# rapidsai/cugraph-gnn

Measured on AMD Instinct MI355X. Metric: sampled-edges/sec (sample+renumber+feature-gather+SAGEConv fwd), ogbn-products-like fan-out [25, 10], higher is better.
Workload: dtype int64 ids (int32 timed as a variant) + f32 features (SAGE lin_l/lin_r product: bf16x3-split MFMA, f32 accumulate); 1 GPU; ogbn-products-like RMAT: V=2449029, E=118462496 directed (CSR row_ptr i64 / col i64 replicated per GPU), feat fp32 [V,100], batch 1024/GPU, fan-out [25, 10], 2-layer SAGEConv(mean) 100-256-47 fwd, step = 8 call groups of 188 mini-batches; parallelism=dp1 (seeds sharded, no data-path collective)

## Files before the change

cugraph-gnn_amd/csrc/wg_append_unique.hip:

```cpp
#include <algorithm>
#include <type_traits>

#include "wg_common.hpp"

namespace wgamd {
namespace {

constexpr int kEmptyPos = 0x7fffffff;

template <typename KeyT>
struct key_traits;
template <>
struct key_traits<int32_t> {
  using cas_t                             = unsigned int;
  static constexpr wholememory_dtype_t dt = WHOLEMEMORY_DT_INT;
};
template <>
struct key_traits<int64_t> {
  using cas_t                             = unsigned long long;
  static constexpr wholememory_dtype_t dt = WHOLEMEMORY_DT_INT64;
};

__device__ __forceinline__ uint32_t hash_key(uint64_t k)
{
// ... 285 lines not shown
  table_clear_packed_kernel<<<(int)std::min<int64_t>(ceil_div(slots, 1024), 4096), 256, 0, stream>>>(table, slots, T, E);
  if (P > 0)
    table_insert_packed_kernel<TgtT, NbrT><<<ceil_div(P, 256), 256, 0, stream>>>(targets, T, neighbors, E, bv, table, slots, lay,
                                                                                 slot_of);
  if (E.host > 0) first_flag_packed_kernel<<<ceil_div(E.host, 256), 256, 0, stream>>>(table, slot_of, T, E, lay, rank);
  WG_HIP_CHECK(hipGetLastError());
  exclusive_scan_i32(rank, rank, E.host, scan_tmp, stream, E.dev);
}

#ifndef WG_LDS_SLOTS
#define WG_LDS_SLOTS 10000
#define WG_LDS_KEYS 3000
#define WG_LDS_THREADS 512
#define WG_LDS_UNROLL 7
#endif
constexpr int kLdsSlots      = WG_LDS_SLOTS;
constexpr int kLdsKeysTarget = WG_LDS_KEYS;
constexpr int kLdsProbeLimit = 256;
constexpr int kLdsThreads    = WG_LDS_THREADS;
constexpr int kLdsMaxRanges  = 2048;
constexpr int kLdsStack      = 40;
constexpr int kLdsChunks     = 16;
constexpr int kBucketThreads = 256;
constexpr int kBucketUnroll  = 4;
constexpr int kLdsUnroll     = WG_LDS_UNROLL;

__device__ __forceinline__ uint32_t hash_id32(uint32_t h)
{
  h ^= h >> 16;
  h *= 0x85ebca6bu;
  h ^= h >> 13;
  h *= 0xc2b2ae35u;
  return h ^ (h >> 16);
}
template <bool ID32>
__device__ __forceinline__ uint32_t hash_id(int64_t id)
{
  if constexpr (ID32) return hash_id32((uint32_t)id);
  else return hash_key((uint64_t)id);
}

struct batch_part {
  int t0, nT, e0, nE, P, R, rb, chunk;
  __device__ batch_part(const batch_view& bv, int b, int keys_target)
  {
    t0 = bv.target_seg[b];
// ... 5 lines not shown
    rb = (t0 + e0) / keys_target + 2 * b;
    chunk = (P + kLdsChunks - 1) / kLdsChunks;
  }
};

__device__ __forceinline__ bool batch_of_block(int G, int parts, int& b, int& part)
{
  const int x = blockIdx.x & 7, y = blockIdx.x >> 3;
  b    = (y / parts) * 8 + x;
  part = y % parts;
  return b < G;
}
inline int batch_grid(int G, int parts) { return 8 * ((G + 7) / 8) * parts; }

struct sort_scratch {
  int keys_target;
  int* seg_off;
  unsigned long long* words;
};

template <typename TgtT, typename NbrT>
__global__ void __launch_bounds__(kBucketThreads)
bucket_sort_kernel(const TgtT* __restrict__ targets, dev_count T_, const NbrT* __restrict__ neighbors, batch_view bv,
                   packed_layout lay, sort_scratch sc)
{
  constexpr bool ID32  = sizeof(NbrT) == 4;
  constexpr int kItems = kLdsMaxRanges / kBucketThreads;
  __shared__ int hist[kLdsMaxRanges];
  __shared__ int wave_tot[kBucketThreads / 64];
  int b, c;
  if (!batch_of_block(bv.G, kLdsChunks, b, c)) return;
  const batch_part bp(bv, b, sc.keys_target);
  if (bp.nE <= 0) return;
  const int T = T_.get(), tid = threadIdx.x;
  for (int r = tid; r < bp.R; r += kBucketThreads) hist[r] = 0;
  __syncthreads();
  const int begin = min(c * bp.chunk, bp.P), end = min(bp.P, begin + bp.chunk);
  const TgtT* tg = targets + bp.t0;
  const NbrT* nb = neighbors + bp.e0 - bp.nT;
  for (int i0 = begin + tid; i0 < end; i0 += kBucketThreads * kBucketUnroll) {
    int64_t id[kBucketUnroll];
#pragma unroll
    for (int k = 0; k < kBucketUnroll; k++) {
      const int i = min(i0 + k * kBucketThreads, end - 1);
      id[k]       = i < bp.nT ? (int64_t)tg[i] : (int64_t)nb[i];
    }
#pragma unroll
    for (int k = 0; k < kBucketUnroll; k++)
      if (i0 + k * kBucketThreads < end) atomicAdd(&hist[__umulhi(hash_id<ID32>(id[k]), (uint32_t)bp.R)], 1);
  }
  __syncthreads();
  {
// ... 31 lines not shown
  unsigned long long* out = sc.words + (bp.t0 + bp.e0) + begin;
  for (int i0 = begin + tid; i0 < end; i0 += kBucketThreads * kBucketUnroll) {
    int64_t id[kBucketUnroll];
#pragma unroll
    for (int k = 0; k < kBucketUnroll; k++) {
      const int i = min(i0 + k * kBucketThreads, end - 1);
      id[k]       = i < bp.nT ? (int64_t)tg[i] : (int64_t)nb[i];
    }
#pragma unroll
    for (int k = 0; k < kBucketUnroll; k++) {
      const int i = i0 + k * kBucketThreads;
      if (i < end) {
        const int dst = atomicAdd(&hist[__umulhi(hash_id<ID32>(id[k]), (uint32_t)bp.R)], 1);
        const int pos = i < bp.nT ? bp.t0 + i : T + bp.e0 + (i - bp.nT);
        out[dst]      = ((unsigned long long)id[k] << lay.pos_bits) | (unsigned long long)pos;
      }
    }
  }
}

template <bool ID32>
__global__ void __launch_bounds__(kLdsThreads)
renumber_lds_kernel(dev_count T_, dev_count E_, batch_view bv, packed_layout lay, int wg_per_batch, sort_scratch sc,
                    int* __restrict__ slot_of, int* __restrict__ tile_sums, int n_tile_sums)
{
  __shared__ unsigned long long tbl[kLdsSlots];
  __shared__ unsigned long long st_lo[kLdsStack], st_span[kLdsStack];
  __shared__ int st_n, overfull;
  __shared__ int seg_base[kLdsChunks], seg_pre[kLdsChunks + 1];
  const unsigned long long kEmpty = ~0ull;
  const int T = T_.get();
  const int tid = threadIdx.x;
  if (blockIdx.x == 0) {
    for (int i = tid; i < n_tile_sums; i += kLdsThreads) tile_sums[i] = 0;
  }
  int b, j;
  if (!batch_of_block(bv.G, wg_per_batch, b, j)) return;
  const batch_part bp(bv, b, sc.keys_target);
  if (bp.nE <= 0) return;
  const unsigned long long pos_mask = lay.pos_mask();
  const volatile int* overfull_now  = &overfull;
  static_assert(kLdsChunks == 16, "the segment search below is written for 16 segments");

  for (int r = j; r < bp.R; r += wg_per_batch) {
    __syncthreads();
    if (tid < kLdsChunks) {
      const int* row = sc.seg_off + (int64_t)(bp.rb + r) * kLdsChunks;
      const int lo = row[tid], n = row[kLdsChunks + tid] - lo;
      seg_base[tid] = bp.t0 + bp.e0 + tid * bp.chunk + lo;
      int inc = n;
#pragma unroll
      for (int d = 1; d < kLdsChunks; d <<= 1) {
        const int up = __shfl_up(inc, d, 64);
        if (tid >= d) inc += up;
      }
      seg_pre[tid + 1] = inc;
      if (tid == 0) {
        seg_pre[0] = 0;
        const unsigned long long lo_h = (((unsigned long long)r << 32) + bp.R - 1) / (unsigned)bp.R;
        st_lo[0]   = lo_h;
        st_span[0] = ((((unsigned long long)(r + 1) << 32) + bp.R - 1) / (unsigned)bp.R) - lo_h;
        st_n       = 1;
// ... 62 lines not shown
            memo[k] = (int)s;
          }
        }
      }
      __syncthreads();
      if (overfull) {
        if (tid == 0) {
          const unsigned long long half = span / 2;
          const int m = st_n;
          if (span < 2 || m + 2 > kLdsStack) __builtin_trap();
          st_lo[m]       = lo + half;
          st_span[m]     = span - half;
          st_lo[m + 1]   = lo;
          st_span[m + 1] = half;
          st_n           = m + 2;
        }
        __syncthreads();
        continue;
      }
      if (one_trip) {
#pragma unroll
        for (int k = 0; k < kLdsUnroll; k++) {
          const int p = (int)(w[k] & pos_mask);
          if (memo[k] >= 0 && p >= T) slot_of[p] = (int)(tbl[memo[k]] & pos_mask);
        }
        __syncthreads();
        continue;
      }
      for (int i0 = 0; i0 < n_pairs; i0 += kLdsThreads * kLdsUnroll) {
        if (!one_trip) {
#pragma unroll
          for (int k = 0; k < kLdsUnroll; k++) w[k] = pair_at(i0 + k * kLdsThreads + tid);
        }
#pragma unroll
        for (int k = 0; k < kLdsUnroll; k++) {
          const unsigned long long word = w[k];
          const unsigned long long id   = word >> lay.pos_bits;
          const int p                   = (int)(word & pos_mask);
          const uint32_t h              = hash_id<ID32>((int64_t)id);
          if (word != kEmpty && p >= T && (unsigned long long)h - lo < span) {
            uint32_t s = __umulhi(h * 0x9E3779B1u, (uint32_t)kLdsSlots);
            unsigned long long cur = tbl[s];
            while ((cur >> lay.pos_bits) != id) {
              s   = s + 1 == (uint32_t)kLdsSlots ? 0u : s + 1;
              cur = tbl[s];
            }
            slot_of[p] = (int)(cur & pos_mask);
          }
        }
      }
      __syncthreads();
    }
  }
}

struct rank_array {
  const int* rank;
  __device__ __forceinline__ int at(int q) const { return rank[q]; }
  __device__ __forceinline__ int total(int , int e_host) const { return rank[e_host]; }
};
struct rank_bits {
  const int* prefix;
  const unsigned long long* words;
  __device__ __forceinline__ int at(int q) const
  {
    const int w = q >> 6;
    return prefix[w] + __popcll(words[w] & ((1ull << (q & 63)) - 1ull));
  }
  __device__ __forceinline__ int total(int e_live, int ) const { return at(e_live); }
};
struct rank_bits_layout {
  int nw;
  int words_at;
  int live_at;
  __host__ __device__ explicit rank_bits_layout(int e_host)
// ... 105 lines not shown
    for (int k = 0; k < kEmitUnroll; k++) row[k] = first[k] < T ? first[k] + shift : tail_row + rank.at(first[k] - T);
#pragma unroll
    for (int k = 0; k < kEmitUnroll; k++) {
      const int i = i0 + k * 256;
      if (i >= end) break;
      const int e = e0 + i;
      if (first[k] == T + e) {
        const KeyT id      = (KeyT)neighbors[e];
        unique_out[row[k]] = id;
        if (bv.unique_batch) bv.unique_batch[row[k]] = b;
        if (bv.frontier_out) {
          const int r = row[k] - tail_row;
          static_cast<KeyT*>(bv.frontier_out)[r] = id;
          bv.frontier_batch_out[r]               = b;
        }
      }
      if (map_out) map_out[e] = row[k];
      if (bv.neighbor_local_out) bv.neighbor_local_out[e] = row[k] - (t0 + shift);
      if (bv.center_local_out) bv.center_local_out[e] = bv.edge_row[e] - s0 + local0;
    }
  }
}

inline int64_t lds_range_records(int64_t capacity_positions, int G) { return capacity_positions / kLdsKeysTarget + 3 * (int64_t)G + 2; }
inline int lds_keys_target()
{
  static const int v = [] {
    const char* e = getenv("WGAMD_RENUMBER_KEYS_TARGET");
    const long t  = e ? atol(e) : 0;
    return t > kLdsKeysTarget ? (int)std::min<long>(t, 1 << 30) : kLdsKeysTarget;
  }();
  return v;
}
inline bool lds_scratch_fits(int64_t capacity_positions, int G, int64_t slots)
{
  return 8 * capacity_positions + 256 <= 8 * slots && lds_range_records(capacity_positions, G) * kLdsChunks <= slots;
}

inline bool lds_path_taken(dev_count T, dev_count E, bool nbr64, const batch_view& bv, int64_t slots, packed_layout& lay)
{
  static const bool no_lds = getenv("WGAMD_RENUMBER_NO_LDS") != nullptr;
  const int64_t bound = bv.id_bound > 0 ? bv.id_bound : (nbr64 ? 0 : ((int64_t)1 << 31));
  const bool batched  = bv.target_batch != nullptr;
  return batched && !no_lds && bv.target_seg && bv.edge_offsets && bv.G > 1 && E.host >= 64 &&
         rank_bits_layout(E.host).ints() <= E.host + 1 &&
         packed_layout_for((int64_t)T.host + E.host, 1, bound, lay) && lds_scratch_fits((int64_t)T.host + E.host, bv.G, slots);
}

template <typename TgtT, typename NbrT>
void prepare_lds_t(const TgtT* targets, dev_count T, const NbrT* neighbors, dev_count E, batch_view bv, packed_layout lay,
                   void* keys, int* minpos, int* slot_of, int* rank, int* scan_tmp, hipStream_t stream)
{
  if (E.host > 0) {
    const int64_t cap = (int64_t)T.host + E.host;
    sort_scratch sc;
    sc.keys_target = lds_keys_target();
    sc.seg_off     = minpos;
    sc.words       = static_cast<unsigned long long*>(keys);
    bucket_sort_kernel<TgtT, NbrT><<<batch_grid(bv.G, kLdsChunks), kBucketThreads, 0, stream>>>(targets, T, neighbors, bv, lay, sc);
    const int64_t per_batch = (cap + bv.G - 1) / bv.G;
    const int wg_per_batch  = (int)std::max<int64_t>(1, std::min<int64_t>((per_batch + kLdsKeysTarget - 1) / kLdsKeysTarget, 32));
    const rank_bits_layout rl(E.host);
    const int n_tiles = (int)((rl.nw + kScanTile - 1) / kScanTile);
    renumber_lds_kernel<sizeof(NbrT) == 4><<<batch_grid(bv.G, wg_per_batch), kLdsThreads, 0, stream>>>(T, E, bv, lay, wg_per_batch, sc,
                                                                                                     slot_of, scan_tmp, n_tiles);
    const int bits_grid = (int)std::min<int64_t>(((int64_t)rl.nw + kBitsWordsPerBlock - 1) / kBitsWordsPerBlock, 256 * 8);
    first_bits_kernel<<<bits_grid, 256, 0, stream>>>(slot_of, T, E, rank, scan_tmp);
    WG_HIP_CHECK(hipGetLastError());
    exclusive_scan_i32_presummed(rank, rank, rl.nw, scan_tmp, stream, rank + rl.live_at);
  }
}

template <typename TgtT, typename NbrT, typename TableKeyT>
void prepare_t(const TgtT* targets, dev_count T, const NbrT* neighbors, dev_count E, batch_view bv, TableKeyT* keys,
               int* minpos, int64_t slots, int* slot_of, int* rank, int* scan_tmp, hipStream_t stream)
{
  const int P = T.host + E.host;
  table_clear_kernel<TableKeyT><<<(int)std::min<int64_t>(ceil_div(slots, 1024), 4096), 256, 0, stream>>>(keys, minpos, slots, T,
                                                                                                   E);
  if (P > 0)
    table_insert_kernel<TgtT, NbrT, TableKeyT><<<ceil_div(P, 256), 256, 0, stream>>>(targets, T, neighbors, E, bv, keys,
                                                                                    minpos, slots, slot_of);
  if (E.host > 0) first_flag_kernel<<<ceil_div(E.host, 256), 256, 0, stream>>>(minpos, slot_of, T, E, rank);
  WG_HIP_CHECK(hipGetLastError());
  exclusive_scan_i32(rank, rank, E.host, scan_tmp, stream, E.dev);
}

template <typename F>
// ... 38 lines not shown
    if constexpr (sizeof(TgtT) == 4) {
      if (!batched) {
        prepare_t<int32_t, int32_t, int32_t>(t, T, n, E, bv, static_cast<int32_t*>(keys), minpos, slots, slot_of, rank, scan_tmp, stream);
        return;
      }
    }
    prepare_t(t, T, n, E, bv, static_cast<int64_t*>(keys), minpos, slots, slot_of, rank, scan_tmp, stream);
  });
}

void append_unique_emit_enqueue(const void* targets, dev_count T, bool tgt64, const void* neighbors, dev_count E, bool nbr64,
                                batch_view bv, const int* minpos, const int* slot_of, const int* rank, int64_t slots,
                                void* unique_out, int* map_out, int* counts_out, hipStream_t stream)
{
  packed_layout lay_unused{};
  const bool bits = lds_path_taken(T, E, nbr64, bv, slots, lay_unused);
  const int P    = T.host + E.host;
  const int grid = ceil_div(P > bv.G + 1 ? P : bv.G + 1, 256);
  const bool per_batch = bv.target_batch != nullptr && bv.target_seg && bv.edge_offsets && bv.G > 1;
  const int bgrid = std::max(batch_grid(bv.G, kEmitChunks), ceil_div(bv.G + 1, 256));
  with_id_types(tgt64, nbr64, targets, neighbors, [&](auto* t, auto* n) {
    using TgtT = std::remove_cv_t<std::remove_pointer_t<decltype(t)>>;
    using NbrT = std::remove_cv_t<std::remove_pointer_t<decltype(n)>>;
    if (per_batch && bits) {
      const rank_bits_layout rl(E.host);
      const rank_bits rb{rank, reinterpret_cast<const unsigned long long*>(rank + rl.words_at)};
      renumber_emit_batched_kernel<TgtT, NbrT, rank_bits><<<bgrid, 256, 0, stream>>>(t, n, slot_of, rb, T, E, bv,
                                                                                    static_cast<TgtT*>(unique_out), map_out, counts_out);
    } else if (per_batch)
      renumber_emit_batched_kernel<TgtT, NbrT, rank_array><<<bgrid, 256, 0, stream>>>(t, n, slot_of, rank_array{rank}, T, E, bv,
                                                                                     static_cast<TgtT*>(unique_out), map_out, counts_out);
    else
      renumber_emit_kernel<TgtT, NbrT><<<grid, 256, 0, stream>>>(t, n, minpos, slot_of, rank, T, E, bv, static_cast<TgtT*>(unique_out),
                                                                map_out, counts_out);
  });
  WG_HIP_CHECK(hipGetLastError());
}

}

extern "C" {

wholememory_error_code_t graph_append_unique(wholememory_tensor_t target_nodes_tensor,
                                             wholememory_tensor_t neighbor_nodes_tensor,
                                             void* output_unique_node_memory_context,
                                             wholememory_tensor_t output_neighbor_raw_to_unique_mapping_tensor,
                                             wholememory_env_func_t* p_env_fns, void* stream)
// ... 61 lines not shown
```

cugraph-gnn_amd/csrc/wg_common.hpp:

```cpp
#pragma once
#include <hip/hip_runtime.h>

#include <cstdarg>
#include <cstdint>
#include <cstdio>
#include <stdexcept>
#include <vector>
#include <mutex>
#include <string>
#include <unordered_map>

#include "wgamd_ops.h"
#include "wgamd_tensor.h"
#include "wgamd_types.h"

struct wholememory_tensor_ {
  void* storage_ptr;
  wholememory_tensor_description_t desc;
  wholememory_tensor_* root;
  wholememory_handle_t handle;
  bool owns_handle = false;
  uint64_t handle_serial = 0;
};

// ... 255 lines not shown
                             const void* seeds, bool seeds64, dev_count n, int M, rng_plan random_seed, const int* offsets,
                             int* big_list, uint32_t* slab, int64_t slab_len, void* dst, int* src_lid,
                             int64_t* edge_gid, hipStream_t stream);
int64_t append_unique_slots(int64_t capacity);
struct batch_view {
  const int* target_batch;
  const int* target_seg;
  const int* edge_row;
  const int* edge_offsets;
  int G;
  int64_t id_bound;
  int* unique_batch;
  int* unique_seg;
  const int* sample_batch;
  const int* sample_seg;
  const int* sample_local0;
  void* frontier_out;
  int* frontier_batch_out;
  int* frontier_seg_out;
  int* frontier_local0_out;
  int* neighbor_local_out;
  int* center_local_out;
  int no_pad;
  __host__ __device__ const int* sbatch() const { return sample_batch ? sample_batch : target_batch; }
  __host__ __device__ const int* sseg() const { return sample_seg ? sample_seg : target_seg; }
};
void append_unique_prepare_enqueue(const void* targets, dev_count T, bool tgt64, const void* neighbors, dev_count E, bool nbr64,
                                   batch_view bv, void* keys, int* minpos, int64_t slots, int* slot_of, int* rank,
                                   int* scan_tmp, hipStream_t stream);
void append_unique_emit_enqueue(const void* targets, dev_count T, bool tgt64, const void* neighbors, dev_count E, bool nbr64,
                                batch_view bv, const int* minpos, const int* slot_of, const int* rank, int64_t slots,
                                void* unique_out, int* map_out, int* counts_out ,
                                hipStream_t stream);


void local_rows_gather(const char* table, wholememory_matrix_description_t tm, const void* idx,
                       wholememory_dtype_t idx_dtype, int64_t n, char* out, wholememory_matrix_description_t om,
                       hipStream_t stream);
void local_rows_scatter(const char* in, wholememory_matrix_description_t im, const void* idx,
                        wholememory_dtype_t idx_dtype, int64_t n, char* table, wholememory_matrix_description_t tm,
                        hipStream_t stream);
void local_rows_permute(const char* src, wholememory_matrix_description_t sm, const int64_t* src_idx, const int64_t* dst_idx,
                        int64_t n, char* dst, wholememory_matrix_description_t dm, hipStream_t stream);
struct id_exchange {
  wholememory_comm_t comm = nullptr;
  int W = 1, me = 0;
// ... 28 lines not shown
```

cugraph-gnn_amd/csrc/wg_fused.hip:

```cpp
#include <atomic>

#include "wg_common.hpp"
#include "wgamd_ext.h"

namespace wgamd {
namespace {

inline size_t align_up(size_t v) { return (v + 255) & ~(size_t)255; }

struct hop_workspace {
  size_t cnt, scan_tmp, nbr, keys, minpos, slot_of, rank, big_list, slab, row_start, row_deg, loc_hist, total;
  int64_t slots, slab_len;
};

hop_workspace plan(int64_t target_cap, int64_t edge_cap, size_t id_bytes, bool batched, int64_t max_row_len = 0)
{
  hop_workspace w{};
  size_t off = 0;
  auto take  = [&](size_t bytes) {
    size_t at = off;
    off += align_up(bytes);
    return at;
  };
  w.slots        = append_unique_slots(target_cap + edge_cap);
// ... 463 lines not shown

wholememory_error_code_t wgamd_sample_hop_batched_nosync(
  const int64_t* csr_row_ptr, const void* csr_col, wholememory_dtype_t id_dtype, const void* targets,
  const int* target_batch, const int* target_seg, int n_batches, int64_t target_cap, int max_sample_count,
  const unsigned long long* random_seeds_dev, int* offsets, int* neighbor_row, int* center_row, int64_t* edge_gid,
  int64_t edge_cap, void* unique, int* unique_batch, int* unique_seg, int* counts_dev, void* workspace,
  size_t workspace_bytes, int64_t n_vertices, void* stream)
{
  return wgamd_sample_hop_batched_nosync_ex(csr_row_ptr, csr_col, id_dtype, targets, target_batch, target_seg, n_batches,
                                            target_cap, max_sample_count, random_seeds_dev, offsets, neighbor_row, center_row,
                                            edge_gid, edge_cap, unique, unique_batch, unique_seg, counts_dev, workspace,
                                            workspace_bytes, n_vertices, 0u, stream);
}

wholememory_error_code_t wgamd_sample_hop_batched_nosync_ex(
  const int64_t* csr_row_ptr, const void* csr_col, wholememory_dtype_t id_dtype, const void* targets,
  const int* target_batch, const int* target_seg, int n_batches, int64_t target_cap, int max_sample_count,
  const unsigned long long* random_seeds_dev, int* offsets, int* neighbor_row, int* center_row, int64_t* edge_gid,
  int64_t edge_cap, void* unique, int* unique_batch, int* unique_seg, int* counts_dev, void* workspace,
  size_t workspace_bytes, int64_t n_vertices, unsigned flags, void* stream)
{
  using namespace wgamd;
  return guarded("wgamd_sample_hop_batched_nosync", [&] {
    WG_REQUIRE_INPUT((flags & ~(WGAMD_HOP_NO_UNIQUE_PAD | WGAMD_HOP_COL_INT32)) == 0, "unknown flag bits");
    WG_REQUIRE_INPUT(!(flags & WGAMD_HOP_COL_INT32) || (id_dtype == WHOLEMEMORY_DT_INT64 && n_vertices > 0 &&
                                                        n_vertices < ((int64_t)1 << 31)),
                     "WGAMD_HOP_COL_INT32 needs INT64 ids and 0 < n_vertices < 2^31");
    WG_REQUIRE_INPUT(target_batch && target_seg && random_seeds_dev && center_row && unique_seg && counts_dev,
                     "null pointer");
    WG_REQUIRE_INPUT(n_batches >= 1 && n_batches < (1 << 20), "bad batch count");
    hop_args a{};
    a.csr_row_ptr = csr_row_ptr; a.csr_col = csr_col; a.id_dtype = id_dtype; a.targets = targets;
    a.n_targets_dev = target_seg + n_batches;
    a.target_cap = target_cap; a.M = max_sample_count;
    a.rng = rng_plan{0, random_seeds_dev, target_batch, target_seg};
    a.bv.target_batch = target_batch; a.bv.target_seg = target_seg; a.bv.G = n_batches;
    a.bv.id_bound = n_vertices > 0 ? n_vertices : 0;
    a.bv.unique_batch = unique_batch; a.bv.unique_seg = unique_seg;
    a.bv.no_pad = (flags & WGAMD_HOP_NO_UNIQUE_PAD) ? 1 : 0;
    a.col32     = (flags & WGAMD_HOP_COL_INT32) != 0;
    a.offsets = offsets; a.neighbor_row = neighbor_row; a.center_row = center_row; a.edge_gid = edge_gid;
    a.edge_cap = edge_cap; a.unique = unique; a.counts_dev = counts_dev; a.workspace = workspace;
    a.workspace_bytes = workspace_bytes; a.stream = static_cast<hipStream_t>(stream);
    run_hop(a);
  });
}

wholememory_error_code_t wgamd_call_group_target_rows(const int* unique_seg, const int* target_seg, const int* target_batch,
                                                      int64_t n_targets, int64_t* rows, void* stream)
{
  using namespace wgamd;
  return guarded("wgamd_call_group_target_rows", [&] {
    WG_REQUIRE_INPUT(n_targets >= 0 && n_targets < ((int64_t)1 << 31), "bad target count");
    if (n_targets == 0) return;
    WG_REQUIRE_INPUT(unique_seg && target_seg && target_batch && rows, "null pointer");
    target_rows_kernel<<<ceil_div(n_targets, 256), 256, 0, static_cast<hipStream_t>(stream)>>>(unique_seg, target_seg, target_batch,
                                                                                              (int)n_targets, rows);
    WG_HIP_CHECK(hipGetLastError());
  });
}

wholememory_error_code_t wgamd_call_group_hop_rows(const int* offsets, const int* frontier_batch, const int* frontier_seg,
// ... 45 lines not shown
  using namespace wgamd;
  return guarded("wgamd_sample_hop_pyg_nosync", [&] {
    WG_REQUIRE_INPUT(p != nullptr, "null parameter block");
    WG_REQUIRE_INPUT(p->nodes && p->node_batch && p->node_seg && p->frontier && p->frontier_batch && p->frontier_seg &&
                       p->frontier_local0 && p->random_seeds_dev && p->center_local && p->neighbor_local &&
                       p->nodes_out && p->nodes_out_batch && p->nodes_out_seg && p->frontier_out &&
                       p->frontier_out_batch && p->frontier_out_seg && p->frontier_out_local0 && p->counts_dev &&
                       p->center_row_scratch,
                     "null pointer");
    WG_REQUIRE_INPUT(p->n_batches >= 1 && p->n_batches < (1 << 20), "bad batch count");
    hop_args a{};
    a.csr_row_ptr = p->csr_row_ptr; a.csr_col = p->csr_col; a.id_dtype = p->id_dtype;
    a.targets = p->nodes; a.n_targets_dev = p->node_seg + p->n_batches; a.target_cap = p->node_cap;
    a.sample_targets = p->frontier; a.n_sample_dev = p->frontier_seg + p->n_batches; a.sample_cap = p->frontier_cap;
    a.M = p->max_sample_count;
    a.rng = rng_plan{0, p->random_seeds_dev, p->frontier_batch, p->frontier_seg};
    a.bv.target_batch = p->node_batch; a.bv.target_seg = p->node_seg; a.bv.G = p->n_batches;
    a.bv.id_bound = p->n_vertices > 0 ? p->n_vertices : 0;
    a.bv.sample_batch = p->frontier_batch; a.bv.sample_seg = p->frontier_seg; a.bv.sample_local0 = p->frontier_local0;
    a.bv.unique_batch = p->nodes_out_batch; a.bv.unique_seg = p->nodes_out_seg;
    a.bv.frontier_out = p->frontier_out; a.bv.frontier_batch_out = p->frontier_out_batch;
    a.bv.frontier_seg_out = p->frontier_out_seg; a.bv.frontier_local0_out = p->frontier_out_local0;
    a.bv.neighbor_local_out = p->neighbor_local; a.bv.center_local_out = p->center_local;
    WG_REQUIRE_INPUT((p->flags & ~(WGAMD_HOP_NO_UNIQUE_PAD | WGAMD_HOP_COL_INT32)) == 0, "unknown flag bits");
    WG_REQUIRE_INPUT(!(p->flags & WGAMD_HOP_COL_INT32) || (p->id_dtype == WHOLEMEMORY_DT_INT64 && p->n_vertices > 0 &&
                                                           p->n_vertices < ((int64_t)1 << 31)),
                     "WGAMD_HOP_COL_INT32 needs INT64 ids and 0 < n_vertices < 2^31");
    a.bv.no_pad = (p->flags & WGAMD_HOP_NO_UNIQUE_PAD) ? 1 : 0;
    a.col32     = (p->flags & WGAMD_HOP_COL_INT32) != 0;
    a.offsets = p->offsets; a.neighbor_row = p->neighbor_row_scratch; a.center_row = p->center_row_scratch;
    a.edge_gid = p->edge_gid; a.edge_cap = p->edge_cap; a.unique = p->nodes_out; a.counts_dev = p->counts_dev;
    a.workspace = p->workspace; a.workspace_bytes = p->workspace_bytes; a.stream = static_cast<hipStream_t>(stream);
    if (p->csr_weight != nullptr) {
      WG_REQUIRE_INPUT(p->weight_dtype == WHOLEMEMORY_DT_FLOAT || p->weight_dtype == WHOLEMEMORY_DT_DOUBLE,
                       "csr_weight must be FLOAT or DOUBLE");
      a.csr_weight = p->csr_weight; a.weight64 = p->weight_dtype == WHOLEMEMORY_DT_DOUBLE; a.max_row_len = p->max_row_len;
    }
    WG_REQUIRE_INPUT(a.neighbor_row != nullptr, "neighbor_row_scratch is NULL");
    run_hop(a);
  });
}

}
```

cugraph-gnn_amd/wholegraph_amd/fused.py:

```python
from dataclasses import dataclass, field
from typing import List, Sequence, Union

import torch

from . import _lib as L
from .env import get_stream, torch_dtype_to_wm


HOP_NO_UNIQUE_PAD = 1
HOP_COL_INT32 = 2

_COL32 = {}


def compact_columns(col: torch.Tensor, n_vertices: int):
    import weakref
    if col.dtype != torch.int64 or not (0 < int(n_vertices) < (1 << 31)) or not col.is_cuda:
        return None
    key = (col.data_ptr(), col.numel())
    hit = _COL32.get(key)
    if hit is not None and hit[0]() is col:
        return hit[1]
    for k in [k for k, v in _COL32.items() if v[0]() is None]:
        del _COL32[k]
    c32 = col.to(torch.int32)
    _COL32[key] = (weakref.ref(col), c32)
    return c32


@dataclass
class WalkResult:

    hops: int
# ... 88 lines not shown
    for s_ in segs_per_hop:
        shift.append([offs[b] + before[b] - s_[b] for b in range(G)])
        before = [before[b] + s_[b + 1] - s_[b] for b in range(G)]
    meta = torch.tensor([[s_[b + 1] - s_[b] for b in range(G)] for s_ in segs_per_hop] + shift, dtype=torch.int64).to(dev)
    batches = torch.arange(G, device=dev)
    merged = [torch.empty(offs[G], dtype=live[0][i].dtype, device=dev) for i in range(n_fields)]
    for h in range(H):
        n_h = segs_per_hop[h][G] - segs_per_hop[h][0]
        if n_h == 0:
            continue
        b_of = torch.repeat_interleave(batches, meta[h], output_size=n_h)
        dest = torch.arange(segs_per_hop[h][0], segs_per_hop[h][G], device=dev) + meta[H + h][b_of]
        for i in range(n_fields):
            merged[i][dest] = live[h][i]
    return merged, offs


class NoSyncWalk:
    def __init__(self, csr_row_ptr: torch.Tensor, csr_col_ind: torch.Tensor, batch_size: int,
                 max_neighbors: List[int], id_dtype=torch.int64, n_batches: int = 1, pad_unique: bool = True,
                 compact_col: bool = True):
        assert csr_row_ptr.is_cuda and csr_col_ind.is_cuda
        assert all(m > 0 for m in max_neighbors), "the no-sync walk needs positive fan-outs"
        self.flags = 0 if pad_unique else HOP_NO_UNIQUE_PAD
        assert csr_col_ind.dtype == id_dtype, "no-sync walk: seeds and csr_col must share a dtype"
        self.row_ptr, self.col = csr_row_ptr, csr_col_ind
        self.n_vertices = int(csr_row_ptr.shape[0]) - 1
        c32 = compact_columns(csr_col_ind, self.n_vertices) if compact_col else None
        if c32 is not None:
            self.col, self.flags = c32, self.flags | HOP_COL_INT32
        self.fanouts = list(max_neighbors)
        self.id_dtype = id_dtype
        self.wm_dtype = torch_dtype_to_wm(id_dtype)
        self.G, self.B = int(n_batches), int(batch_size)
        dev = csr_row_ptr.device
        self.target_caps, self.edge_caps = [], []
        t = self.G * self.B
        for m in self.fanouts:
            self.target_caps.append(t)
            self.edge_caps.append(t * m)
            t = t + t * m
        assert t < (1 << 30), "call group too large: lower n_batches"
        lib = L.lib()
        ws = max(lib.wgamd_sample_hop_workspace_bytes(tc, ec, self.wm_dtype)
                 for tc, ec in zip(self.target_caps, self.edge_caps))
        self.workspace = torch.empty(ws + 256, dtype=torch.uint8, device=dev)
        self.ws_off = (-self.workspace.data_ptr()) % 256
# ... 246 lines not shown
                     for nc, fc, ec in zip(self.node_caps, self.frontier_caps, self.edge_caps))
        else:
            ws = max(lib.wgamd_sample_hop_weighted_workspace_bytes(max(nc, fc), ec, self.wm_dtype, self.max_row_len)
                     for nc, fc, ec in zip(self.node_caps, self.frontier_caps, self.edge_caps))
        self.workspace = torch.empty(ws + 256, dtype=torch.uint8, device=dev)
        self.ws_off, self.ws_bytes, self.dev = (-self.workspace.data_ptr()) % 256, ws, dev
        self.seed_seg = (torch.arange(self.G + 1, dtype=torch.int32, device=dev) * self.B).contiguous()
        self.seed_batch = torch.arange(self.G, dtype=torch.int32, device=dev).repeat_interleave(self.B).contiguous()
        self.zeros_g = torch.zeros(self.G, dtype=torch.int32, device=dev)

    def run(self, seeds: torch.Tensor, random_seeds, seed_seg: torch.Tensor = None, seed_batch: torch.Tensor = None) -> PygWalkResult:
        assert seeds.dtype == self.id_dtype and seeds.shape[0] == self.G * self.B
        assert (seed_seg is None) == (seed_batch is None)
        lib, dev, G = L.lib(), self.dev, self.G
        hops = len(self.fanout)
        if isinstance(random_seeds, torch.Tensor):
            rs = random_seeds.to(device=dev, dtype=torch.int64).contiguous()
        else:
            rs = torch.tensor([[v - (1 << 64) if v & (1 << 63) else v for v in (int(x) & 0xFFFFFFFFFFFFFFFF for x in row)]
                               for row in random_seeds], dtype=torch.int64, device=dev)
        assert rs.shape == (hops, G)
        res = PygWalkResult(hops, G, self.B, counts=torch.empty((hops, 2), dtype=torch.int32, device=dev))
        res._keepalive = [rs]
        if seed_seg is None:
            seed_seg, seed_batch = self.seed_seg, self.seed_batch
        else:
            assert seed_seg.dtype == torch.int32 and seed_seg.shape[0] == G + 1 and seed_seg.is_contiguous()
            assert seed_batch.dtype == torch.int32 and seed_batch.shape[0] == G * self.B and seed_batch.is_contiguous()
        nodes, n_batch, n_seg = seeds, seed_batch, seed_seg
        front, f_batch, f_seg, f_local0 = seeds, seed_batch, seed_seg, self.zeros_g
        i32 = dict(dtype=torch.int32, device=dev)
        for k, (m, fc, nc, ec) in enumerate(zip(self.fanout, self.frontier_caps, self.node_caps, self.edge_caps)):
            offsets = torch.empty(fc + 1, **i32)
            row_l, col_l = torch.empty(ec, **i32), torch.empty(ec, **i32)
            scratch_r, scratch_c = torch.empty(ec, **i32), torch.empty(ec, **i32)
            gid = torch.empty(ec, dtype=torch.int64, device=dev)
            nodes_out = torch.empty(nc + ec, dtype=self.id_dtype, device=dev)
            nodes_out_batch, nodes_out_seg = torch.empty(nc + ec, **i32), torch.empty(G + 1, **i32)
            f_out = torch.empty(ec, dtype=self.id_dtype, device=dev)
            f_out_batch, f_out_seg, f_out_l0 = torch.empty(ec, **i32), torch.empty(G + 1, **i32), torch.empty(G, **i32)
            p = _PygHop(self.row_ptr.data_ptr(), self.col.data_ptr(), self.wm_dtype, G, m, rs[k].data_ptr(),
                        nodes.data_ptr(), n_batch.data_ptr(), n_seg.data_ptr(), nc,
                        front.data_ptr(), f_batch.data_ptr(), f_seg.data_ptr(), f_local0.data_ptr(), fc,
                        offsets.data_ptr(), row_l.data_ptr(), col_l.data_ptr(), gid.data_ptr(), ec,
                        nodes_out.data_ptr(), nodes_out_batch.data_ptr(), nodes_out_seg.data_ptr(),
                        f_out.data_ptr(), f_out_batch.data_ptr(), f_out_seg.data_ptr(), f_out_l0.data_ptr(),
                        res.counts[k].data_ptr(), scratch_r.data_ptr(), scratch_c.data_ptr(),
                        self.workspace.data_ptr() + self.ws_off, self.ws_bytes,
                        None if self.weight is None else self.weight.data_ptr(),
                        0 if self.weight is None else torch_dtype_to_wm(self.weight.dtype), self.max_row_len,
                        int(self.row_ptr.shape[0]) - 1, self.flags)
            L.check(lib.wgamd_sample_hop_pyg_nosync(_ct.byref(p), get_stream()), "wgamd_sample_hop_pyg_nosync")
            res.offsets.append(offsets)
            res.row_local.append(row_l)
            res.col_local.append(col_l)
            res.edge_gid.append(gid)
            res.frontier_seg.append(f_seg)
            res.frontier_batch.append(f_batch)
            res.frontier_local0.append(f_local0)
            res._keepalive += [scratch_r, scratch_c, f_batch, n_batch, front, f_local0]
            nodes, n_batch, n_seg = nodes_out, nodes_out_batch, nodes_out_seg
            front, f_batch, f_seg, f_local0 = f_out, f_out_batch, f_out_seg, f_out_l0
        res.frontier_seg.append(f_seg)
        res.nodes, res.node_seg = nodes, n_seg
        return res


class HeteroPygWalk:

    def __init__(self, graphs, batch_size: int, fanout, n_batches: int, biased: bool = False, num_nodes=None,
                 pad_unique: bool = True):
        self.flags = 0 if pad_unique else HOP_NO_UNIQUE_PAD
        self.biased = bool(biased)
        self.num_nodes = dict(num_nodes) if num_nodes else {}
# ... 56 lines not shown
        return ids.contiguous(), b.to(torch.int32).contiguous(), f_seg, st["begin"].contiguous()

    def run(self, seed_type: str, seeds: torch.Tensor, random_seeds: torch.Tensor, seed_lists=None):
        lib, dev, G = L.lib(), self.dev, self.G
        assert seed_lists is not None or (seeds.dtype == torch.int64 and seeds.shape[0] == G * self.B and seeds.is_cuda)
        rs = random_seeds.to(device=dev, dtype=torch.int64).contiguous()
        assert rs.shape == (self.hops * len(self.etypes), G)
        i32 = dict(dtype=torch.int32, device=dev)
        state = {}
        for t in self.ntypes:
            state[t] = dict(nodes=torch.zeros(1, dtype=torch.int64, device=dev), batch=torch.zeros(1, **i32),
                            seg=self.zeros_g1, cap=0, begin=self.zeros_g, gained_cap=0)
        if seed_lists is None:
            state[seed_type] = dict(nodes=seeds, batch=self.seed_batch, seg=self.seed_seg, cap=G * self.B,
                                    begin=self.zeros_g, gained_cap=G * self.B)
        else:
            for t, (ids, seg, batch) in seed_lists.items():
                assert ids.dtype == torch.int64 and seg.dtype == torch.int32 and batch.dtype == torch.int32
                assert seg.shape[0] == G + 1 and batch.shape[0] == ids.shape[0]
                state[t] = dict(nodes=ids.contiguous(), batch=batch.contiguous(), seg=seg.contiguous(), cap=int(ids.shape[0]),
                                begin=self.zeros_g, gained_cap=int(ids.shape[0]))
        rec = dict(calls=[], sizes=[{t: (state[t]["seg"][1:] - state[t]["seg"][:-1]) for t in self.ntypes}])
        keep = [rs]
        for h in range(self.hops):
            fronts = {t: (self._frontier(state[t], state[t]["gained_cap"]) if state[t]["gained_cap"] > 0 else None)
                      for t in self.ntypes}
            f_caps = {t: state[t]["gained_cap"] for t in self.ntypes}
            for t in self.ntypes:
                st = state[t]
                st["begin"] = (st["seg"][1:] - st["seg"][:-1]).to(torch.int32).contiguous()
                st["gained_cap"] = 0
            for ti, et in enumerate(self.etypes):
                src_t, _, dst_t = et
                m, fr = self.fanout[et][h], fronts[dst_t]
                if m == 0 or fr is None:
                    rec["calls"].append(None)
                    continue
                g = self.graphs[et]
                f_ids, f_batch, f_seg, f_l0 = fr
                fc = f_caps[dst_t]
                ec = fc * m
                st = state[src_t]
                nc = max(st["cap"], 1)
                offsets = torch.empty(fc + 1, **i32)
                row_l, col_l = torch.empty(ec, **i32), torch.empty(ec, **i32)
                scratch_r, scratch_c = torch.empty(ec, **i32), torch.empty(ec, **i32)
                gid = torch.empty(ec, dtype=torch.int64, device=dev)
                nodes_out = torch.empty(nc + ec, dtype=torch.int64, device=dev)
                nodes_out_batch, nodes_out_seg = torch.empty(nc + ec, **i32), torch.empty(G + 1, **i32)
                f_out = torch.empty(ec, dtype=torch.int64, device=dev)
                f_out_batch, f_out_seg, f_out_l0 = torch.empty(ec, **i32), torch.empty(G + 1, **i32), torch.empty(G, **i32)
                counts = torch.empty(2, **i32)
                mrl = self.max_row_len.get(et, 0)
                ws_ptr, ws_bytes = self._workspace(max(nc, fc), ec, mrl)
                c32 = self.col32[et]
                p = _PygHop(g.row_ptr.data_ptr(), (g.col if c32 is None else c32).data_ptr(), self.wm_dtype, G, m,
                            rs[h * len(self.etypes) + ti].data_ptr(),
                            st["nodes"].data_ptr(), st["batch"].data_ptr(), st["seg"].data_ptr(), nc,
                            f_ids.data_ptr(), f_batch.data_ptr(), f_seg.data_ptr(), f_l0.data_ptr(), fc,
                            offsets.data_ptr(), row_l.data_ptr(), col_l.data_ptr(), gid.data_ptr(), ec,
                            nodes_out.data_ptr(), nodes_out_batch.data_ptr(), nodes_out_seg.data_ptr(),
                            f_out.data_ptr(), f_out_batch.data_ptr(), f_out_seg.data_ptr(), f_out_l0.data_ptr(),
                            counts.data_ptr(), scratch_r.data_ptr(), scratch_c.data_ptr(), ws_ptr, ws_bytes,
                            g.weight.data_ptr() if self.biased else None,
                            torch_dtype_to_wm(g.weight.dtype) if self.biased else 0, mrl,
                            int(self.num_nodes.get(src_t, 0)),
                            self.flags | (0 if c32 is None else HOP_COL_INT32))
                L.check(lib.wgamd_sample_hop_pyg_nosync(_ct.byref(p), get_stream()), "wgamd_sample_hop_pyg_nosync")
                keep += [scratch_r, scratch_c, f_out, f_out_batch, f_out_seg, f_out_l0, counts, f_ids, f_batch, f_l0,
                         st["nodes"], st["batch"], st["seg"]]
                rec["calls"].append(dict(et=et, offsets=offsets, row=row_l, col=col_l, gid=gid, f_seg=f_seg, f_batch=f_batch,
                                         f_local0=f_l0, frontier_cap=fc, hop=h, counts=counts))
                st["nodes"], st["batch"], st["seg"] = nodes_out, nodes_out_batch, nodes_out_seg
                st["cap"] = nc + ec
                st["gained_cap"] += ec
            rec["sizes"].append({t: (state[t]["seg"][1:] - state[t]["seg"][:-1]) for t in self.ntypes})
        rec["state"], rec["keep"] = state, keep
        return rec

    def finalize_batches(self, rec):
        G, dev = self.G, self.dev
        state = rec["state"]
        pieces = [state[t]["seg"] for t in self.ntypes]
        pieces += [s_[t] for s_ in rec["sizes"] for t in self.ntypes]
        live_calls = [c for c in rec["calls"] if c is not None]
        pieces += [c["offsets"][c["f_seg"].long()] for c in live_calls]
        flat = torch.cat([p_.reshape(-1).to(torch.int64) for p_ in pieces]).cpu().tolist()
        host, at = [], 0
        for p_ in pieces:
            host.append(flat[at:at + p_.numel()])
# ... 39 lines not shown
```

include/wgamd_ext.h:

```cpp
#ifndef WGAMD_EXT_H_
#define WGAMD_EXT_H_

#include "wgamd_types.h"

#ifdef __cplusplus
extern "C" {
#endif


wholememory_error_code_t wgamd_spmm_csr_f32(const int* row_ptr,
                                            const int* col,
                                            int64_t n_rows,
                                            const float* x,
                                            int64_t ldx,
                                            int F,
                                            const void* src_ids,
                                            wholememory_dtype_t src_ids_dtype,
                                            int mean,
                                            float* out,
                                            int64_t ldo,
                                            void* stream);

wholememory_error_code_t wgamd_sage_aggregate_f32(const int* row_ptr,
                                                  const int* col,
// ... 108 lines not shown
                                                         const void* targets,
                                                         const int* target_batch,
                                                         const int* target_seg,
                                                         int n_batches,
                                                         int64_t target_cap,
                                                         int max_sample_count,
                                                         const unsigned long long* random_seeds_dev,
                                                         int* offsets,
                                                         int* neighbor_row,
                                                         int* center_row,
                                                         int64_t* edge_gid,
                                                         int64_t edge_cap,
                                                         void* unique,
                                                         int* unique_batch,
                                                         int* unique_seg,
                                                         int* counts_dev,
                                                         void* workspace,
                                                         size_t workspace_bytes,
                                                         int64_t n_vertices ,
                                                         void* stream);

#define WGAMD_HOP_NO_UNIQUE_PAD 1u
#define WGAMD_HOP_COL_INT32 2u

wholememory_error_code_t wgamd_sample_hop_batched_nosync_ex(const int64_t* csr_row_ptr,
                                                         const void* csr_col,
                                                         wholememory_dtype_t id_dtype,
                                                         const void* targets,
                                                         const int* target_batch,
                                                         const int* target_seg,
                                                         int n_batches,
                                                         int64_t target_cap,
                                                         int max_sample_count,
                                                         const unsigned long long* random_seeds_dev,
                                                         int* offsets,
                                                         int* neighbor_row,
                                                         int* center_row,
                                                         int64_t* edge_gid,
                                                         int64_t edge_cap,
                                                         void* unique,
                                                         int* unique_batch,
                                                         int* unique_seg,
                                                         int* counts_dev,
                                                         void* workspace,
                                                         size_t workspace_bytes,
                                                         int64_t n_vertices ,
// ... 382 lines not shown
```

Measured before the change: 5.521 billion sampled-edges/s.

## Rank new unique ids per batch in LDS instead of global bit-scan

When batches have uniform edge capacity, the renumber kernel now counts newly seen ids per batch, and a new emit kernel builds first-occurrence bitmaps and prefix ranks in shared memory for each batch's edge window. This replaces the global first-bits kernel and exclusive scan over all edges with a small cross-batch prefix over per-batch counts. It adds a fallback flag for batches exceeding the cap, an extra flag bit set by default from Python, and dynamic LDS up to 64KB per block.

```diff
diff --git a/cugraph-gnn_amd/csrc/wg_append_unique.hip b/cugraph-gnn_amd/csrc/wg_append_unique.hip
--- a/cugraph-gnn_amd/csrc/wg_append_unique.hip
+++ b/cugraph-gnn_amd/csrc/wg_append_unique.hip
@@ -331,6 +331,7 @@
 constexpr int kLdsStack      = 40;
 constexpr int kLdsChunks     = 16;
 constexpr int kBucketThreads = 256;
+constexpr int kNewStride     = 16;
 constexpr int kBucketUnroll  = 4;
 constexpr int kLdsUnroll     = WG_LDS_UNROLL;
 
@@ -382,12 +383,15 @@
 template <typename TgtT, typename NbrT>
 __global__ void __launch_bounds__(kBucketThreads)
 bucket_sort_kernel(const TgtT* __restrict__ targets, dev_count T_, const NbrT* __restrict__ neighbors, batch_view bv,
-                   packed_layout lay, sort_scratch sc)
+                   packed_layout lay, sort_scratch sc, int* __restrict__ batch_new)
 {
   constexpr bool ID32  = sizeof(NbrT) == 4;
   constexpr int kItems = kLdsMaxRanges / kBucketThreads;
   __shared__ int hist[kLdsMaxRanges];
   __shared__ int wave_tot[kBucketThreads / 64];
+  if (blockIdx.x == 0 && batch_new) {
+    for (int i = threadIdx.x; i <= bv.G * kNewStride; i += kBucketThreads) batch_new[i] = 0;
+  }
   int b, c;
   if (!batch_of_block(bv.G, kLdsChunks, b, c)) return;
   const batch_part bp(bv, b, sc.keys_target);
@@ -465,11 +469,11 @@
 template <bool ID32>
 __global__ void __launch_bounds__(kLdsThreads)
 renumber_lds_kernel(dev_count T_, dev_count E_, batch_view bv, packed_layout lay, int wg_per_batch, sort_scratch sc,
-                    int* __restrict__ slot_of, int* __restrict__ tile_sums, int n_tile_sums)
+                    int* __restrict__ slot_of, int* __restrict__ tile_sums, int n_tile_sums, int* __restrict__ batch_new)
 {
   __shared__ unsigned long long tbl[kLdsSlots];
   __shared__ unsigned long long st_lo[kLdsStack], st_span[kLdsStack];
-  __shared__ int st_n, overfull;
+  __shared__ int st_n, overfull, new_cnt;
   __shared__ int seg_base[kLdsChunks], seg_pre[kLdsChunks + 1];
   const unsigned long long kEmpty = ~0ull;
   const int T = T_.get();
@@ -481,6 +485,8 @@
   if (!batch_of_block(bv.G, wg_per_batch, b, j)) return;
   const batch_part bp(bv, b, sc.keys_target);
   if (bp.nE <= 0) return;
+  if (batch_new && j == 0 && tid == 0 && bp.nE > bv.batch_edge_cap) batch_new[bv.G * kNewStride] = 1;
+  int n_new = 0;
   const unsigned long long pos_mask = lay.pos_mask();
   const volatile int* overfull_now  = &overfull;
   static_assert(kLdsChunks == 16, "the segment search below is written for 16 segments");
@@ -589,7 +595,11 @@
 #pragma unroll
         for (int k = 0; k < kLdsUnroll; k++) {
           const int p = (int)(w[k] & pos_mask);
-          if (memo[k] >= 0 && p >= T) slot_of[p] = (int)(tbl[memo[k]] & pos_mask);
+          if (memo[k] >= 0 && p >= T) {
+            const int first = (int)(tbl[memo[k]] & pos_mask);
+            slot_of[p]      = first;
+            n_new += first == p;
+          }
         }
         __syncthreads();
         continue;
@@ -612,12 +622,23 @@
               s   = s + 1 == (uint32_t)kLdsSlots ? 0u : s + 1;
               cur = tbl[s];
             }
-            slot_of[p] = (int)(cur & pos_mask);
+            const int first = (int)(cur & pos_mask);
+            slot_of[p]      = first;
+            n_new += first == p;
           }
         }
       }
       __syncthreads();
     }
+  }
+  if (batch_new) {
+    if (tid == 0) new_cnt = 0;
+    __syncthreads();
+#pragma unroll
+    for (int d = 32; d > 0; d >>= 1) n_new += __shfl_down(n_new, d, 64);
+    if ((tid & 63) == 0 && n_new) atomicAdd(&new_cnt, n_new);
+    __syncthreads();
+    if (tid == 0 && new_cnt) atomicAdd(&batch_new[b * kNewStride], new_cnt);
   }
 }
 
@@ -769,6 +790,177 @@
   }
 }
 
+#ifndef WG_RANK_PARTS
+#define WG_RANK_PARTS 2
+#define WG_RANK_THREADS 1024
+#endif
+constexpr int kRankParts       = WG_RANK_PARTS;
+constexpr int kRankThreads     = WG_RANK_THREADS;
+constexpr int kRankWaves       = kRankThreads / 64;
+constexpr int kRankUnroll      = 8;
+constexpr int kRankWindowBytes = 65536;
+__host__ __device__ inline int rank_window_words(int batch_edge_cap) { return batch_edge_cap / 64 + 1; }
+inline size_t rank_window_bytes(int batch_edge_cap) { return (size_t)rank_window_words(batch_edge_cap) * 12; }
+
+template <typename TgtT, typename NbrT>
+__global__ void __launch_bounds__(kRankThreads)
+renumber_emit_ranked_kernel(const TgtT* __restrict__ targets, const NbrT* __restrict__ neighbors,
+                            const int* __restrict__ slot_of, const int* __restrict__ batch_new, dev_count T_, dev_count E_,
+                            batch_view bv, TgtT* __restrict__ unique_out, int* __restrict__ map_out,
+                            int* __restrict__ counts_out)
+{
+  using KeyT = TgtT;
+  extern __shared__ unsigned long long rank_window[];
+  __shared__ int red_before[kRankWaves], red_all[kRankWaves], wave_tot[kRankWaves];
+  const int nw_cap          = rank_window_words(bv.batch_edge_cap);
+  unsigned long long* words = rank_window;
+  int* pre                  = reinterpret_cast<int*>(rank_window + nw_cap);
+  const int T = T_.get(), E = E_.get();
+  const int tid = threadIdx.x, lane = tid & 63, wave = tid >> 6;
+  const int gtid = blockIdx.x * kRankThreads + tid, gsize = gridDim.x * kRankThreads;
+  int b, c;
+  const bool mine = batch_of_block(bv.G, kRankParts, b, c);
+  int shift = 0, U = 0;
+  {
+    int before = 0, all = 0;
+    for (int g = tid; g < bv.G; g += kRankThreads) {
+      const int v = batch_new[g * kNewStride];
+      all += v;
+      before += g < b ? v : 0;
+    }
+#pragma unroll
+    for (int d = 32; d > 0; d >>= 1) {
+      before += __shfl_down(before, d, 64);
+      all += __shfl_down(all, d, 64);
+    }
+    if (lane == 0) {
+      red_before[wave] = before;
+      red_all[wave]    = all;
+    }
+    __syncthreads();
+#pragma unroll
+    for (int w = 0; w < kRankWaves; w++) {
+      shift += red_before[w];
+      U += red_all[w];
+    }
+  }
+  if (batch_new[bv.G * kNewStride] != 0) {
+    if (gtid == 0 && counts_out) {
+      counts_out[0] = E;
+      counts_out[1] = -1;
+    }
+    return;
+  }
+  if (gtid == 0) {
+    if (counts_out) {
+      counts_out[0] = E;
+      counts_out[1] = T + U;
+    }
+    if (bv.unique_seg) {
+      bv.unique_seg[bv.G] = bv.target_seg[bv.G] + U;
+      if (bv.frontier_seg_out) bv.frontier_seg_out[bv.G] = U;
+    }
+  }
+  if (counts_out && !bv.no_pad)
+    for (int p = T + U + gtid; p < T_.host + E_.host; p += gsize) unique_out[p] = (KeyT)-1;
+  if (!mine) return;
+
+  const int t0 = bv.target_seg[b], nT = bv.target_seg[b + 1] - t0;
+  const int s0 = bv.sseg()[b];
+  const int e0 = bv.edge_offsets[s0], nE = bv.edge_offsets[bv.sseg()[b + 1]] - e0;
+  const int tail_row = t0 + nT + shift;
+  const int local0   = bv.sample_local0 ? bv.sample_local0[b] : 0;
+  if (c == 0 && tid == 0 && bv.unique_seg) {
+    bv.unique_seg[b] = t0 + shift;
+    if (bv.frontier_seg_out) bv.frontier_seg_out[b] = shift;
+    if (bv.frontier_local0_out) bv.frontier_local0_out[b] = nT;
+  }
+  {
+    const int chunk = (nT + kRankParts - 1) / kRankParts;
+    const int end   = min(nT, (c + 1) * chunk);
+    for (int i = c * chunk + tid; i < end; i += kRankThreads) {
+      unique_out[t0 + i + shift] = targets[t0 + i];
+      if (bv.unique_batch) bv.unique_batch[t0 + i + shift] = b;
+    }
+  }
+  const int chunk = (nE + kRankParts - 1) / kRankParts;
+  const int begin = c * chunk, end = min(nE, begin + chunk);
+  if (begin >= end) return;
+  const int* first_of = slot_of + T + e0;
+  const int p0        = T + e0;
+  const int nw = (end + 63) >> 6;
+  for (int w0 = wave; w0 < nw; w0 += kRankWaves * kRankUnroll) {
+    int first[kRankUnroll];
+#pragma unroll
+    for (int k = 0; k < kRankUnroll; k++) {
+      const int i = (w0 + k * kRankWaves) * 64 + lane;
+      first[k]    = i < nE ? first_of[i] : -1;
+    }
+#pragma unroll
+    for (int k = 0; k < kRankUnroll; k++) {
+      const int w = w0 + k * kRankWaves;
+      const unsigned long long word = __ballot(first[k] == p0 + w * 64 + lane);
+      if (lane == 0 && w < nw) {
+        words[w] = word;
+        pre[w]   = __popcll(word);
+      }
+    }
+  }
+  __syncthreads();
+  {
+    const int per = (nw + kRankThreads - 1) / kRankThreads;
+    const int lo = min(tid * per, nw), hi = min(lo + per, nw);
+    int sum = 0;
+    for (int w = lo; w < hi; w++) sum += pre[w];
+    int inc = sum;
+#pragma unroll
+    for (int d = 1; d < 64; d <<= 1) {
+      const int up = __shfl_up(inc, d, 64);
+      if (lane >= d) inc += up;
+    }
+    if (lane == 63) wave_tot[wave] = inc;
+    __syncthreads();
+    int run = inc - sum;
+    for (int w = 0; w < wave; w++) run += wave_tot[w];
+    for (int w = lo; w < hi; w++) {
+      const int v = pre[w];
+      pre[w]      = run;
+      run += v;
+    }
+  }
+  __syncthreads();
+  for (int i0 = begin + tid; i0 < end; i0 += kRankThreads * kEmitUnroll) {
+    int first[kEmitUnroll], row[kEmitUnroll];
+#pragma unroll
+    for (int k = 0; k < kEmitUnroll; k++) first[k] = first_of[min(i0 + k * kRankThreads, end - 1)];
+#pragma unroll
+    for (int k = 0; k < kEmitUnroll; k++) {
+      const int q = max(first[k] - p0, 0);
+      row[k]      = first[k] < T ? first[k] + shift
+                                 : tail_row + pre[q >> 6] + __popcll(words[q >> 6] & ((1ull << (q & 63)) - 1ull));
+    }
+#pragma unroll
+    for (int k = 0; k < kEmitUnroll; k++) {
+      const int i = i0 + k * kRankThreads;
+      if (i >= end) break;
+      const int e = e0 + i;
+      if (first[k] == T + e) {
+        const KeyT id      = (KeyT)neighbors[e];
+        unique_out[row[k]] = id;
+        if (bv.unique_batch) bv.unique_batch[row[k]] = b;
+        if (bv.frontier_out) {
+          const int r = row[k] - (t0 + nT);
+          static_cast<KeyT*>(bv.frontier_out)[r] = id;
+          bv.frontier_batch_out[r]               = b;
+        }
+      }
+      if (map_out) map_out[e] = row[k];
+      if (bv.neighbor_local_out) bv.neighbor_local_out[e] = row[k] - (t0 + shift);
+      if (bv.center_local_out) bv.center_local_out[e] = bv.edge_row[e] - s0 + local0;
+    }
+  }
+}
+
 inline int64_t lds_range_records(int64_t capacity_positions, int G) { return capacity_positions / kLdsKeysTarget + 3 * (int64_t)G + 2; }
 inline int lds_keys_target()
 {
@@ -794,6 +986,11 @@
          packed_layout_for((int64_t)T.host + E.host, 1, bound, lay) && lds_scratch_fits((int64_t)T.host + E.host, bv.G, slots);
 }
 
+inline bool batch_ranks_taken(dev_count E, const batch_view& bv)
+{
+  return bv.batch_edge_cap > 0 && (int64_t)bv.G * kNewStride <= E.host && rank_window_bytes(bv.batch_edge_cap) <= (size_t)kRankWindowBytes;
+}
+
 template <typename TgtT, typename NbrT>
 void prepare_lds_t(const TgtT* targets, dev_count T, const NbrT* neighbors, dev_count E, batch_view bv, packed_layout lay,
                    void* keys, int* minpos, int* slot_of, int* rank, int* scan_tmp, hipStream_t stream)
@@ -804,13 +1001,20 @@
     sc.keys_target = lds_keys_target();
     sc.seg_off     = minpos;
     sc.words       = static_cast<unsigned long long*>(keys);
-    bucket_sort_kernel<TgtT, NbrT><<<batch_grid(bv.G, kLdsChunks), kBucketThreads, 0, stream>>>(targets, T, neighbors, bv, lay, sc);
+    const bool per_batch_ranks = batch_ranks_taken(E, bv);
+    int* batch_new             = per_batch_ranks ? rank : nullptr;
+    bucket_sort_kernel<TgtT, NbrT><<<batch_grid(bv.G, kLdsChunks), kBucketThreads, 0, stream>>>(targets, T, neighbors, bv, lay, sc,
+                                                                                                batch_new);
     const int64_t per_batch = (cap + bv.G - 1) / bv.G;
     const int wg_per_batch  = (int)std::max<int64_t>(1, std::min<int64_t>((per_batch + kLdsKeysTarget - 1) / kLdsKeysTarget, 32));
     const rank_bits_layout rl(E.host);
-    const int n_tiles = (int)((rl.nw + kScanTile - 1) / kScanTile);
+    const int n_tiles = per_batch_ranks ? 0 : (int)((rl.nw + kScanTile - 1) / kScanTile);
     renumber_lds_kernel<sizeof(NbrT) == 4><<<batch_grid(bv.G, wg_per_batch), kLdsThreads, 0, stream>>>(T, E, bv, lay, wg_per_batch, sc,
-                                                                                                     slot_of, scan_tmp, n_tiles);
+                                                                                                     slot_of, scan_tmp, n_tiles, batch_new);
+    if (per_batch_ranks) {
+      WG_HIP_CHECK(hipGetLastError());
+      return;
+    }
     const int bits_grid = (int)std::min<int64_t>(((int64_t)rl.nw + kBitsWordsPerBlock - 1) / kBitsWordsPerBlock, 256 * 8);
     first_bits_kernel<<<bits_grid, 256, 0, stream>>>(slot_of, T, E, rank, scan_tmp);
     WG_HIP_CHECK(hipGetLastError());
@@ -895,7 +1099,10 @@
   with_id_types(tgt64, nbr64, targets, neighbors, [&](auto* t, auto* n) {
     using TgtT = std::remove_cv_t<std::remove_pointer_t<decltype(t)>>;
     using NbrT = std::remove_cv_t<std::remove_pointer_t<decltype(n)>>;
-    if (per_batch && bits) {
+    if (per_batch && bits && batch_ranks_taken(E, bv)) {
+      renumber_emit_ranked_kernel<TgtT, NbrT><<<batch_grid(bv.G, kRankParts), kRankThreads, rank_window_bytes(bv.batch_edge_cap), stream>>>(
+        t, n, slot_of, rank, T, E, bv, static_cast<TgtT*>(unique_out), map_out, counts_out);
+    } else if (per_batch && bits) {
       const rank_bits_layout rl(E.host);
       const rank_bits rb{rank, reinterpret_cast<const unsigned long long*>(rank + rl.words_at)};
       renumber_emit_batched_kernel<TgtT, NbrT, rank_bits><<<bgrid, 256, 0, stream>>>(t, n, slot_of, rb, T, E, bv,
diff --git a/cugraph-gnn_amd/csrc/wg_common.hpp b/cugraph-gnn_amd/csrc/wg_common.hpp
--- a/cugraph-gnn_amd/csrc/wg_common.hpp
+++ b/cugraph-gnn_amd/csrc/wg_common.hpp
@@ -301,6 +301,7 @@
   int* neighbor_local_out;
   int* center_local_out;
   int no_pad;
+  int batch_edge_cap;
   __host__ __device__ const int* sbatch() const { return sample_batch ? sample_batch : target_batch; }
   __host__ __device__ const int* sseg() const { return sample_seg ? sample_seg : target_seg; }
 };
diff --git a/cugraph-gnn_amd/csrc/wg_fused.hip b/cugraph-gnn_amd/csrc/wg_fused.hip
--- a/cugraph-gnn_amd/csrc/wg_fused.hip
+++ b/cugraph-gnn_amd/csrc/wg_fused.hip
@@ -509,7 +509,7 @@
 {
   using namespace wgamd;
   return guarded("wgamd_sample_hop_batched_nosync", [&] {
-    WG_REQUIRE_INPUT((flags & ~(WGAMD_HOP_NO_UNIQUE_PAD | WGAMD_HOP_COL_INT32)) == 0, "unknown flag bits");
+    WG_REQUIRE_INPUT((flags & ~(WGAMD_HOP_NO_UNIQUE_PAD | WGAMD_HOP_COL_INT32 | WGAMD_HOP_UNIFORM_BATCHES)) == 0, "unknown flag bits");
     WG_REQUIRE_INPUT(!(flags & WGAMD_HOP_COL_INT32) || (id_dtype == WHOLEMEMORY_DT_INT64 && n_vertices > 0 &&
                                                         n_vertices < ((int64_t)1 << 31)),
                      "WGAMD_HOP_COL_INT32 needs INT64 ids and 0 < n_vertices < 2^31");
@@ -525,6 +525,7 @@
     a.bv.id_bound = n_vertices > 0 ? n_vertices : 0;
     a.bv.unique_batch = unique_batch; a.bv.unique_seg = unique_seg;
     a.bv.no_pad = (flags & WGAMD_HOP_NO_UNIQUE_PAD) ? 1 : 0;
+    a.bv.batch_edge_cap = (flags & WGAMD_HOP_UNIFORM_BATCHES) ? (int)ceil_div(edge_cap, (int64_t)n_batches) : 0;
     a.col32     = (flags & WGAMD_HOP_COL_INT32) != 0;
     a.offsets = offsets; a.neighbor_row = neighbor_row; a.center_row = center_row; a.edge_gid = edge_gid;
     a.edge_cap = edge_cap; a.unique = unique; a.counts_dev = counts_dev; a.workspace = workspace;
@@ -616,11 +617,12 @@
     a.bv.frontier_out = p->frontier_out; a.bv.frontier_batch_out = p->frontier_out_batch;
     a.bv.frontier_seg_out = p->frontier_out_seg; a.bv.frontier_local0_out = p->frontier_out_local0;
     a.bv.neighbor_local_out = p->neighbor_local; a.bv.center_local_out = p->center_local;
-    WG_REQUIRE_INPUT((p->flags & ~(WGAMD_HOP_NO_UNIQUE_PAD | WGAMD_HOP_COL_INT32)) == 0, "unknown flag bits");
+    WG_REQUIRE_INPUT((p->flags & ~(WGAMD_HOP_NO_UNIQUE_PAD | WGAMD_HOP_COL_INT32 | WGAMD_HOP_UNIFORM_BATCHES)) == 0, "unknown flag bits");
     WG_REQUIRE_INPUT(!(p->flags & WGAMD_HOP_COL_INT32) || (p->id_dtype == WHOLEMEMORY_DT_INT64 && p->n_vertices > 0 &&
                                                            p->n_vertices < ((int64_t)1 << 31)),
                      "WGAMD_HOP_COL_INT32 needs INT64 ids and 0 < n_vertices < 2^31");
     a.bv.no_pad = (p->flags & WGAMD_HOP_NO_UNIQUE_PAD) ? 1 : 0;
+    a.bv.batch_edge_cap = (p->flags & WGAMD_HOP_UNIFORM_BATCHES) ? (int)ceil_div(p->edge_cap, (int64_t)p->n_batches) : 0;
     a.col32     = (p->flags & WGAMD_HOP_COL_INT32) != 0;
     a.offsets = p->offsets; a.neighbor_row = p->neighbor_row_scratch; a.center_row = p->center_row_scratch;
     a.edge_gid = p->edge_gid; a.edge_cap = p->edge_cap; a.unique = p->nodes_out; a.counts_dev = p->counts_dev;
diff --git a/cugraph-gnn_amd/wholegraph_amd/fused.py b/cugraph-gnn_amd/wholegraph_amd/fused.py
--- a/cugraph-gnn_amd/wholegraph_amd/fused.py
+++ b/cugraph-gnn_amd/wholegraph_amd/fused.py
@@ -9,6 +9,7 @@
 
 HOP_NO_UNIQUE_PAD = 1
 HOP_COL_INT32 = 2
+HOP_UNIFORM_BATCHES = 8
 
 _COL32 = {}
 
@@ -143,7 +144,7 @@
                  compact_col: bool = True):
         assert csr_row_ptr.is_cuda and csr_col_ind.is_cuda
         assert all(m > 0 for m in max_neighbors), "the no-sync walk needs positive fan-outs"
-        self.flags = 0 if pad_unique else HOP_NO_UNIQUE_PAD
+        self.flags = (0 if pad_unique else HOP_NO_UNIQUE_PAD) | HOP_UNIFORM_BATCHES
         assert csr_col_ind.dtype == id_dtype, "no-sync walk: seeds and csr_col must share a dtype"
         self.row_ptr, self.col = csr_row_ptr, csr_col_ind
         self.n_vertices = int(csr_row_ptr.shape[0]) - 1
@@ -436,8 +437,10 @@
         assert rs.shape == (hops, G)
         res = PygWalkResult(hops, G, self.B, counts=torch.empty((hops, 2), dtype=torch.int32, device=dev))
         res._keepalive = [rs]
+        flags = self.flags
         if seed_seg is None:
             seed_seg, seed_batch = self.seed_seg, self.seed_batch
+            flags |= HOP_UNIFORM_BATCHES
         else:
             assert seed_seg.dtype == torch.int32 and seed_seg.shape[0] == G + 1 and seed_seg.is_contiguous()
             assert seed_batch.dtype == torch.int32 and seed_batch.shape[0] == G * self.B and seed_batch.is_contiguous()
@@ -463,7 +466,7 @@
                         self.workspace.data_ptr() + self.ws_off, self.ws_bytes,
                         None if self.weight is None else self.weight.data_ptr(),
                         0 if self.weight is None else torch_dtype_to_wm(self.weight.dtype), self.max_row_len,
-                        int(self.row_ptr.shape[0]) - 1, self.flags)
+                        int(self.row_ptr.shape[0]) - 1, flags)
             L.check(lib.wgamd_sample_hop_pyg_nosync(_ct.byref(p), get_stream()), "wgamd_sample_hop_pyg_nosync")
             res.offsets.append(offsets)
             res.row_local.append(row_l)
@@ -566,6 +569,7 @@
                                 begin=self.zeros_g, gained_cap=int(ids.shape[0]))
         rec = dict(calls=[], sizes=[{t: (state[t]["seg"][1:] - state[t]["seg"][:-1]) for t in self.ntypes}])
         keep = [rs]
+        flags = self.flags | (HOP_UNIFORM_BATCHES if seed_lists is None else 0)
         for h in range(self.hops):
             fronts = {t: (self._frontier(state[t], state[t]["gained_cap"]) if state[t]["gained_cap"] > 0 else None)
                       for t in self.ntypes}
@@ -609,7 +613,7 @@
                             g.weight.data_ptr() if self.biased else None,
                             torch_dtype_to_wm(g.weight.dtype) if self.biased else 0, mrl,
                             int(self.num_nodes.get(src_t, 0)),
-                            self.flags | (0 if c32 is None else HOP_COL_INT32))
+                            flags | (0 if c32 is None else HOP_COL_INT32))
                 L.check(lib.wgamd_sample_hop_pyg_nosync(_ct.byref(p), get_stream()), "wgamd_sample_hop_pyg_nosync")
                 keep += [scratch_r, scratch_c, f_out, f_out_batch, f_out_seg, f_out_l0, counts, f_ids, f_batch, f_l0,
                          st["nodes"], st["batch"], st["seg"]]
diff --git a/include/wgamd_ext.h b/include/wgamd_ext.h
--- a/include/wgamd_ext.h
+++ b/include/wgamd_ext.h
@@ -154,6 +154,7 @@
 
 #define WGAMD_HOP_NO_UNIQUE_PAD 1u
 #define WGAMD_HOP_COL_INT32 2u
+#define WGAMD_HOP_UNIFORM_BATCHES 8u
 
 wholememory_error_code_t wgamd_sample_hop_batched_nosync_ex(const int64_t* csr_row_ptr,
                                                          const void* csr_col,
```

Result: faster. 5.643 billion sampled-edges/s, median of 6 (+2.2%).
